# ubc-vision/COTR

Measured on AMD Instinct MI355X. Metric: query-correspondences/sec at 256x512 SBS, 1k queries, higher is better.
Workload: dtype f32

## Files before the change

cotr_amd/_lib.py:

```python
import ctypes
import os

import torch

from .build import LIB, LIB_EXP

c_float_p = ctypes.c_void_p

_PROTOS = {
    'cotr_abi_version': (ctypes.c_int, []),
    'cotr_create': (ctypes.c_int, [ctypes.POINTER(ctypes.c_void_p), ctypes.c_int]),
    'cotr_destroy': (None, [ctypes.c_void_p]),
    'cotr_last_error': (ctypes.c_char_p, [ctypes.c_void_p]),
    'cotr_load_weights': (ctypes.c_int, [ctypes.c_void_p, ctypes.POINTER(ctypes.c_char_p),
                                         ctypes.POINTER(ctypes.c_void_p), ctypes.POINTER(ctypes.c_int64), ctypes.c_int]),
    'cotr_encode': (ctypes.c_int, [ctypes.c_void_p, c_float_p, ctypes.c_int, ctypes.c_void_p]),
    'cotr_backbone': (ctypes.c_int, [ctypes.c_void_p, c_float_p, ctypes.c_int, c_float_p, ctypes.c_void_p]),
    'cotr_backbone_upto': (ctypes.c_int, [ctypes.c_void_p, c_float_p, ctypes.c_int, ctypes.c_int, c_float_p, ctypes.c_void_p]),
    'cotr_decode': (ctypes.c_int, [ctypes.c_void_p, c_float_p, ctypes.c_int, ctypes.c_int, c_float_p, ctypes.c_void_p]),
    'cotr_forward': (ctypes.c_int, [ctypes.c_void_p, c_float_p, c_float_p, ctypes.c_int, ctypes.c_int, c_float_p,
                                    ctypes.c_void_p]),
    'cotr_workspace_bytes': (ctypes.c_int, [ctypes.c_void_p, ctypes.c_int, ctypes.c_int, ctypes.POINTER(ctypes.c_size_t)]),
    'cotr_scratch_bytes': (ctypes.c_int, [ctypes.c_void_p, ctypes.c_int, ctypes.c_int, ctypes.POINTER(ctypes.c_size_t)]),
    'cotr_batch_chunks': (ctypes.c_int, [ctypes.c_void_p, ctypes.c_int, ctypes.c_int, ctypes.c_int, ctypes.POINTER(ctypes.c_int), ctypes.c_int]),
# ... 109 lines not shown
    'cotr_get_knob': (ctypes.c_int, [ctypes.c_void_p, ctypes.c_char_p, ctypes.POINTER(ctypes.c_int), ctypes.POINTER(ctypes.c_int)]),
    'cotr_set_knob': (ctypes.c_int, [ctypes.c_void_p, ctypes.c_char_p, ctypes.c_int]),
    'cotr_check_knob': (ctypes.c_int, [ctypes.c_char_p, ctypes.c_int]),
    'cotr_reset_knobs': (ctypes.c_int, [ctypes.c_void_p]),
    'cotr_is_experimental': (ctypes.c_int, []),
    'cotr_bench_linear': (ctypes.c_int, [c_float_p, c_float_p, c_float_p, c_float_p, ctypes.c_int, ctypes.c_int,
                                         ctypes.c_int, ctypes.c_int, ctypes.c_int, ctypes.POINTER(ctypes.c_float)]),
    'cotr_bench_conv': (ctypes.c_int, [c_float_p, c_float_p, c_float_p, c_float_p, c_float_p] + [ctypes.c_int] * 9 +
                        [ctypes.POINTER(ctypes.c_float)]),
    'cotr_op_linear_cfg': (ctypes.c_int, [c_float_p, c_float_p, c_float_p, c_float_p, ctypes.c_int, c_float_p,
                                          ctypes.c_int, ctypes.c_int, ctypes.c_int, ctypes.c_int, ctypes.c_void_p]),
    'cotr_op_conv_cfg': (ctypes.c_int, [c_float_p, c_float_p, c_float_p, c_float_p, c_float_p, ctypes.c_int, c_float_p] +
                         [ctypes.c_int] * 8 + [ctypes.c_void_p]),
    'cotr_debug_ffn_times': (ctypes.c_int, [ctypes.c_void_p]),
    'cotr_debug_attention_times': (ctypes.c_int, [ctypes.c_void_p]),
    'cotr_gemm_pick_conv': (ctypes.c_int, [ctypes.c_int] * 7),
    'cotr_debug_conv_times': (ctypes.c_int, [c_float_p, c_float_p, c_float_p, c_float_p, c_float_p] + [ctypes.c_int] * 8 +
                              [ctypes.c_void_p, ctypes.c_void_p]),
}

_EXP_PROTOS = {
    'cotr_op_dec_head': (ctypes.c_int, [c_float_p] * 11 + [ctypes.c_int, ctypes.c_int, ctypes.c_int, ctypes.c_void_p]),
    'cotr_op_linear_ln': (ctypes.c_int, [c_float_p] * 7 + [ctypes.c_int, ctypes.c_int, ctypes.c_void_p]),
    'cotr_op_split_h2': (ctypes.c_int, [c_float_p, ctypes.c_void_p, ctypes.c_size_t, ctypes.c_void_p]),
    'cotr_op_unsplit_h2': (ctypes.c_int, [ctypes.c_void_p, c_float_p, ctypes.c_size_t, ctypes.c_void_p]),
    'cotr_op_set_h2_flags': (ctypes.c_int, [ctypes.c_int]),
    'cotr_h2_fallbacks': (ctypes.c_long, []),
    'cotr_op_attention_h2': (ctypes.c_int, [c_float_p, ctypes.c_int, ctypes.c_int, c_float_p, c_float_p, ctypes.c_int, c_float_p, ctypes.c_int,
                                            ctypes.c_int, ctypes.c_int, ctypes.c_int, ctypes.c_void_p]),
}
# ... 88 lines not shown
```

cotr_amd/csrc/api.hip:

```cpp
#include <math.h>
#include <stdio.h>
#include <stdlib.h>
#include <string.h>

#include <algorithm>
#include <map>
#include <string>
#include <vector>

#include <limits.h>

#include "../../include/cotr_hip.h"
#include "common.h"
#include "train.h"

int init_attention_attributes();
void set_ffn_debug_times(unsigned long long* p);
void set_attention_debug_times(unsigned long long* p);

namespace {

constexpr int D = 256, FFN = 1024, TOK = 512, CFEAT = 1024;
constexpr int ENC_CHUNK_MAX = 128;
constexpr int DEC_ROWS = 32768;
constexpr float QSCALE = 0.17677669529663687f;

struct ConvW {
  const float *w, *scale, *bias;
  int cin, cout, k, stride;
};
struct EncW {
  const float *in_w, *in_b, *out_w, *out_b, *l1w, *l1b, *l2w, *l2b, *n1w, *n1b, *n2w, *n2b;
// ... 69 lines not shown
}
KnobSet g_process_knobs = default_knobs();
}
thread_local const KnobSet* cotr_tls_knobs = &g_process_knobs;

struct cotr_ctx {
  int device = 0;
  std::string err;
  KnobSet knobs = default_knobs();
  float* wbuf = nullptr;
  size_t wfloats = 0;
  bool loaded = false;
  std::vector<ConvW> convs;
  struct FusedBlock { const float *w2p = nullptr, *w3p = nullptr, *wdp = nullptr; };
  FusedBlock l1_fused[3];
  const float *ip_w = nullptr, *ip_b = nullptr;
  std::vector<EncW> enc;
  std::vector<DecW> dec;
  const float *kv_w = nullptr, *kv_b = nullptr;
  const float *dn_w = nullptr, *dn_b = nullptr;
  const float* mlp_w[3] = {nullptr, nullptr, nullptr};
  const float* mlp_b[3] = {nullptr, nullptr, nullptr};
  float* pos = nullptr;
  float* tab_qkv = nullptr;
  float* tab_kv = nullptr;
  Arena memkv;
  int enc_B = 0;
  Arena enc_scr, dec_scr;
  std::map<std::string, std::pair<const float*, size_t>> taps;
  bool keep_taps = false;
// ... 414 lines not shown
  h->device = device;
  if (hipMalloc(reinterpret_cast<void**>(&h->pos), (size_t)TOK * D * sizeof(float)) != hipSuccess ||
      launch_pos_table(h->pos, nullptr) != 0 || hipStreamSynchronize(nullptr) != hipSuccess) {
    g_create_error = "building the image position table failed";
    delete h;
    return COTR_ERR_HIP;
  }
  *out = h;
  return COTR_OK;
}

void cotr_destroy(cotr_handle h) {
  if (!h) return;
  DeviceScope scope(h->device);
  (void)hipDeviceSynchronize();
  prof_reset(h);
  if (h->wbuf) (void)hipFree(h->wbuf);
  if (h->pos) (void)hipFree(h->pos);
  for (hipEvent_t ev : {h->ev_fork, h->ev_q, h->ev_mem, h->ev_kv})
    if (ev) (void)hipEventDestroy(ev);
  if (h->side) (void)hipStreamDestroy(h->side);
  for (Arena* a : {&h->memkv, &h->enc_scr, &h->dec_scr})
    if (a->ptr && !a->external) (void)hipFree(a->ptr);
  for (auto& kv : h->tap_store)
    if (kv.second.ptr) (void)hipFree(kv.second.ptr);
  for (auto& st : h->vl_stage) {
    if (st.host) (void)hipHostFree(st.host);
    if (st.ev) (void)hipEventDestroy(st.ev);
  }
  delete h;
// ... 92 lines not shown
      inplanes = planes * 4;
    }
  }
  size_t l1_w2p[3], l1_w3p[3], l1_wdp = 0;
  for (int b = 0; b < 3; ++b) {
    const int c1i = b == 0 ? 1 : 5 + 3 * (b - 1);
    l1_w2p[b] = reserve(36864);
    l1_w3p[b] = reserve(16384);
    bottleneck_pack_w2(&host[convs[c1i + 1].w], &host[l1_w2p[b]]);
    bottleneck_pack_w3(&host[convs[c1i + 2].w], &host[l1_w3p[b]]);
    if (b == 0) {
      l1_wdp = reserve(16384);
      bottleneck_pack_w3(&host[convs[c1i + 3].w], &host[l1_wdp]);
    }
  }
  const size_t ip_w = put("input_proj.weight", (size_t)D * CFEAT), ip_b = put("input_proj.bias", D);

  struct EncOff { size_t v[12]; };
  std::vector<EncOff> enc(n_enc), dec(n_dec);
  for (int i = 0; i < n_enc; ++i) {
    const std::string p = "transformer.encoder.layers." + std::to_string(i) + ".";
    size_t* v = enc[i].v;
    v[0] = put(p + "self_attn.in_proj_weight", (size_t)3 * D * D);
    v[1] = put(p + "self_attn.in_proj_bias", 3 * D);
    v[2] = put(p + "self_attn.out_proj.weight", (size_t)D * D);
    v[3] = put(p + "self_attn.out_proj.bias", D);
    v[4] = put(p + "linear1.weight", (size_t)FFN * D);
    v[5] = put(p + "linear1.bias", FFN);
    v[6] = put(p + "linear2.weight", (size_t)D * FFN);
    v[7] = put(p + "linear2.bias", D);
// ... 46 lines not shown
    h->wbuf = nullptr;
  }
  if (!h->wbuf) {
    HIPCHK(h, hipMalloc(reinterpret_cast<void**>(&h->wbuf), host.size() * sizeof(float)));
    h->wfloats = host.size();
  }
  HIPCHK(h, hipMemcpy(h->wbuf, host.data(), host.size() * sizeof(float), hipMemcpyHostToDevice));
  const float* base = h->wbuf;
  h->convs.clear();
  for (const auto& c : convs) h->convs.push_back({base + c.w, base + c.scale, base + c.bias, c.cin, c.cout, c.k, c.stride});
  for (int b = 0; b < 3; ++b) {
    h->l1_fused[b].w2p = base + l1_w2p[b];
    h->l1_fused[b].w3p = base + l1_w3p[b];
    h->l1_fused[b].wdp = b == 0 ? base + l1_wdp : nullptr;
  }
  h->ip_w = base + ip_w; h->ip_b = base + ip_b;
  h->enc.clear();
  for (const auto& e : enc)
    h->enc.push_back({base + e.v[0], base + e.v[1], base + e.v[2], base + e.v[3], base + e.v[4], base + e.v[5],
                      base + e.v[6], base + e.v[7], base + e.v[8], base + e.v[9], base + e.v[10], base + e.v[11]});
  h->dec.clear();
  for (const auto& e : dec)
    h->dec.push_back({base + e.v[0], base + e.v[1], base + e.v[2], base + e.v[3], base + e.v[4], base + e.v[5],
                      base + e.v[6], base + e.v[7], base + e.v[8], base + e.v[9], base + e.v[10], base + e.v[11]});
  h->kv_w = base + kv_w; h->kv_b = base + kv_b;
  h->dn_w = base + dn_w; h->dn_b = base + dn_b;
  for (int i = 0; i < 3; ++i) { h->mlp_w[i] = base + mw[i]; h->mlp_b[i] = base + mb[i]; }
  h->tab_qkv = h->wbuf + tab_qkv;
  h->tab_kv = h->wbuf + tab_kv;
  for (int l = 0; l < n_enc; ++l)
// ... 1 lines not shown
                       h->tab_qkv + (size_t)l * TOK * 3 * D, TOK, 2 * D, D, nullptr, 3 * D)) return r;
  for (int l = 0; l < n_dec; ++l)
    if (int r = linear(h, h->pos, nullptr, 0, 1, 0, h->kv_w + (size_t)l * 2 * D * D, nullptr, nullptr, 0, 1.f, 0,
                       h->tab_kv + (size_t)l * 2 * D, TOK, D, D, nullptr, n_dec * 2 * D)) return r;
  HIPCHK(h, hipStreamSynchronize(nullptr));
  h->loaded = true;
  h->enc_B = 0;
  return COTR_OK;
}

static int enc_backbone_pass(cotr_ctx* h, const EncBufs& eb, const float* img_c, int Bc, int b0, float* src_out, float* feat_out,
                             int upto, hipStream_t s) {
  int ci = 0;
  if (knob(KN_FUSED_STEM) && !h->keep_taps) {
    const ConvW& c0 = h->convs[ci++];
    KCHK(h, launch_stem_pool(img_c, c0.w, 160, c0.scale, c0.bias, eb.b_pool, Bc, s), "stem_pool");
    prof_mark(h, "stem_pool conv7x7+bn+relu+maxpool", s, 2);
  } else {
    { int r = stem(h, h->convs[ci++], img_c, eb.b_stem, Bc, s); if (r) return r; }
    KCHK(h, launch_maxpool(eb.b_stem, eb.b_pool, Bc, 128, 128, 64, s), "maxpool");
    prof_mark(h, "maxpool", s, 2);
  }
  prof_mark(h, "stem+pool", s);
  if (int r = tap_save(h, "stem", eb.b_stem, ENC_STEM * Bc, s)) return r;
  if (int r = tap_save(h, "pool", eb.b_pool, ENC_POOL * Bc, s)) return r;
  const float* x = eb.b_pool;
  float* outbuf[2] = {eb.b_x, eb.b_y};
  int flip = 0, H = 64, W = 64;
  for (int st = 0; st < 3; ++st) {
    for (int b = 0; b < kStages[st].blocks; ++b) {
      const int stride = (b == 0) ? kStages[st].stride : 1;
// ... 727 lines not shown
  p.A = x; p.lda = Cin; p.W = w; p.C = y; p.ldc = Cout;
  p.scale = scale; p.bias = bias; p.residual = residual; p.ldr = Cout; p.relu = relu;
  return op_ret(launch_gemm(GEMM_CONV, p, static_cast<hipStream_t>(stream)));
}

int cotr_op_stem(const float* img, const float* w, const float* scale, const float* bias, float* y, int B,
                 cotr_stream stream) {
  GemmParams p = base_params();
  p.M = B * 128 * 256; p.N = 64; p.K = 160; p.A = img; p.W = w; p.C = y; p.ldc = 64;
  p.scale = scale; p.bias = bias; p.relu = 1;
  return op_ret(launch_gemm(GEMM_STEM, p, static_cast<hipStream_t>(stream)));
}

int cotr_op_stem_pool(const float* img, const float* w, const float* scale, const float* bias, float* y, int B,
                      cotr_stream stream) {
  return op_ret(launch_stem_pool(img, w, 160, scale, bias, y, B, static_cast<hipStream_t>(stream)));
}

int cotr_op_maxpool(const float* x, float* y, int B, int Hin, int Win, int C, cotr_stream stream) {
  return op_ret(launch_maxpool(x, y, B, Hin, Win, C, static_cast<hipStream_t>(stream)));
}

int cotr_op_attention(const float* q, int ldq, const float* k, const float* v, int ldkv, float* o, int ldo,
                      int nb, int nq, cotr_stream stream) {
  if (init_attention_attributes() != 0) return COTR_ERR_HIP;
  return op_ret(launch_attention(q, ldq, k, v, ldkv, o, ldo, nb, nq, static_cast<hipStream_t>(stream)));
}

int cotr_op_attention_fused(const float* q, int ldq, const float* x, const float* x2, const float* wq, const float* bq,
                            float qscale, const float* k, const float* v, int ldkv, float* o, int ldo, const float* wo,
                            float* part, int nb, int nq, cotr_stream stream) {
// ... 167 lines not shown
  p.A = x; p.lda = Cin; p.W = w; p.C = y; p.ldc = Cout;
  p.scale = scale; p.bias = bias; p.residual = residual; p.ldr = Cout; p.relu = relu;
  return op_ret(launch_gemm_cfg(GEMM_CONV, cfg, p, static_cast<hipStream_t>(stream)));
}

int cotr_debug_ffn_times(unsigned long long* times) {
  set_ffn_debug_times(times);
  return COTR_OK;
}

int cotr_debug_attention_times(unsigned long long* times) {
  set_attention_debug_times(times);
  return COTR_OK;
}

int cotr_gemm_pick_conv(int B, int Hin, int Win, int Cin, int Cout, int ksize, int stride) {
  GemmParams p = base_params();
  const int pad = ksize / 2;
  p.Hin = Hin; p.Win = Win; p.Cin = Cin;
  p.Hout = (Hin + 2 * pad - ksize) / stride + 1;
  p.Wout = (Win + 2 * pad - ksize) / stride + 1;
  p.ksize = ksize; p.stride = stride; p.pad = pad;
  p.M = B * p.Hout * 2 * p.Wout; p.N = Cout; p.K = ksize * ksize * Cin;
  p.lda = Cin; p.ldc = Cout; p.ldr = Cout;
  return gemm_pick_config(GEMM_CONV, p);
}

int cotr_debug_conv_times(const float* x, const float* w, const float* scale, const float* bias, float* y, int B, int Hin, int Win,
                          int Cin, int Cout, int ksize, int stride, int cfg, unsigned long long* times, cotr_stream stream) {
  GemmParams p = base_params();
// ... 192 lines not shown
```

cotr_amd/csrc/bottleneck.hip:

```cpp
#include "common.h"

struct BottleneckParams {
  const float* x;
  float* y;
  const float* w1;
  const float* w2p;
  const float* w3p;
  const float* wdp;
  const float *s1, *b1, *s2, *b2, *s3, *b3, *sd, *bd;
  const float* zeros;
  int B;
};

#define BT_H 64
#define BT_W 64
#define BT_LDT 68

template <int CIN, bool DS>
__global__ __launch_bounds__(512) void bottleneck_kernel(const BottleneckParams p) {
  static_assert(CIN == 64 || CIN == 256, "layer1: 64 (block 0) or 256 input channels");
  static_assert(!DS || CIN == 64, "the downsample branch belongs to block 0");
  constexpr int LDX = CIN + 4;
  constexpr int C4 = CIN / 4;
  constexpr int NX = 64 * C4 / 512;
  extern __shared__ __attribute__((aligned(16))) float smem[];
  float* Xs = smem;
  float* W1s = Xs + 64 * LDX;
  float* T1s = W1s + 64 * LDX;
  float* T2s = T1s + 64 * BT_LDT;
  float* RED = (CIN == 256) ? W1s : T2s + 32 * BT_LDT;

  const int t = threadIdx.x, lane = t & 63;
  const int wave = __builtin_amdgcn_readfirstlane(t >> 6);
  const int l31 = lane & 31, hh = lane >> 5;
  const int bid = blockIdx.x;
  const int tx = bid & 15, ty = (bid >> 4) & 15, b = bid >> 8;
  const int side = tx >> 3, x0 = (tx & 7) * 8, y0 = ty * 4;
  const size_t pair_base = (size_t)b * BT_H * (2 * BT_W);

  f32x4 xr[NX], wr[NX];
#pragma unroll
  for (int i = 0; i < NX; ++i) {
    const int idx = t + 512 * i;
    const int row = idx / C4, c4 = idx % C4;
    const int py = (row * 205) >> 11, px = row - py * 10;
    const int yy = y0 - 1 + py, xx = x0 - 1 + px;
    const bool ok = row < 60 && yy >= 0 && yy < BT_H && xx >= 0 && xx < BT_W;
// ... 12 lines not shown
    for (int j = 0; j < 8; ++j) w3f[j] = w3g[j * 64];
    if constexpr (DS) {
      const f32x4* wdg = reinterpret_cast<const f32x4*>(p.wdp) + (size_t)(wave * 8) * 64 + lane;
#pragma unroll
      for (int j = 0; j < 8; ++j) wdf[j] = wdg[j * 64];
    }
  }
#pragma unroll
  for (int i = 0; i < NX; ++i) {
    const int idx = t + 512 * i;
    const int row = idx / C4, c4 = idx % C4;
    *reinterpret_cast<f32x4*>(&Xs[row * LDX + c4 * 4]) = xr[i];
    *reinterpret_cast<f32x4*>(&W1s[row * LDX + c4 * 4]) = wr[i];
  }
  __syncthreads();

  {
    const int mb = wave & 1, nb = (wave >> 1) & 1, kh = wave >> 2;
    constexpr int NS = CIN / 16;
    f32x16 acc;
#pragma unroll
    for (int r = 0; r < 16; ++r) acc[r] = 0.f;
    const float* ar = &Xs[(32 * mb + l31) * LDX + kh * (CIN / 2) + hh * 4];
    const float* br = &W1s[(32 * nb + l31) * LDX + kh * (CIN / 2) + hh * 4];
#pragma unroll
    for (int j = 0; j < NS; ++j) {
      const f32x4 a = *reinterpret_cast<const f32x4*>(ar + j * 8);
      const f32x4 bb = *reinterpret_cast<const f32x4*>(br + j * 8);
#pragma unroll
      for (int e = 0; e < 4; ++e) acc = __builtin_amdgcn_mfma_f32_32x32x2f32(a[e], bb[e], acc, 0, 0, 0);
// ... 8 lines not shown
      const int ch = 32 * nb + l31;
      const float sc = p.s1[ch], bi = p.b1[ch];
#pragma unroll
      for (int r = 0; r < 16; ++r) {
        const int row = 32 * mb + (r & 3) + 8 * (r >> 2) + 4 * hh;
        const int py = (row * 205) >> 11, px = row - py * 10;
        const int yy = y0 - 1 + py, xx = x0 - 1 + px;
        const bool ok = row < 60 && yy >= 0 && yy < BT_H && xx >= 0 && xx < BT_W;
        float v = acc[r] + RED[((mb * 2 + nb) * 16 + r) * 64 + lane];
        v = fmaf(v, sc, bi);
        v = (v < 0.f) ? 0.f : v;
        T1s[row * BT_LDT + ch] = ok ? v : 0.f;
      }
    }
    __syncthreads();
  }

  {
    f32x16 acc;
#pragma unroll
    for (int r = 0; r < 16; ++r) acc[r] = 0.f;
    const int rowbase = (l31 >> 3) * 10 + (l31 & 7);
#pragma unroll
    for (int i = 0; i < 18; ++i) {
      const int s = 18 * kgB + i;
      const int tap = s >> 3, kc = s & 7;
      const int ky = (tap * 11) >> 5, kx = tap - 3 * ky;
      const f32x4 a = *reinterpret_cast<const f32x4*>(&T1s[(rowbase + ky * 10 + kx) * BT_LDT + kc * 8 + hh * 4]);
#pragma unroll
      for (int e = 0; e < 4; ++e) acc = __builtin_amdgcn_mfma_f32_32x32x2f32(a[e], w2f[i][e], acc, 0, 0, 0);
// ... 3 lines not shown
    __syncthreads();
    const int nb = wave & 1, rg = wave >> 1;
    const int ch = 32 * nb + l31;
    const float sc = p.s2[ch], bi = p.b2[ch];
#pragma unroll
    for (int rr = 0; rr < 4; ++rr) {
      const int r = rg * 4 + rr;
      float v = 0.f;
#pragma unroll
      for (int kg = 0; kg < 4; ++kg) v += RED[((kg * 2 + nb) * 16 + r) * 64 + lane];
      v = fmaf(v, sc, bi);
      v = (v < 0.f) ? 0.f : v;
      T2s[((r & 3) + 8 * (r >> 2) + 4 * hh) * BT_LDT + ch] = v;
    }
    __syncthreads();
  }

  {
    f32x16 acc, accd;
#pragma unroll
    for (int r = 0; r < 16; ++r) acc[r] = accd[r] = 0.f;
#pragma unroll
    for (int j = 0; j < 8; ++j) {
      const f32x4 a = *reinterpret_cast<const f32x4*>(&T2s[l31 * BT_LDT + j * 8 + hh * 4]);
#pragma unroll
      for (int e = 0; e < 4; ++e) acc = __builtin_amdgcn_mfma_f32_32x32x2f32(a[e], w3f[j][e], acc, 0, 0, 0);
    }
    if constexpr (DS) {
      const int crow = ((l31 >> 3) + 1) * 10 + (l31 & 7) + 1;
#pragma unroll
      for (int j = 0; j < 8; ++j) {
        const f32x4 a = *reinterpret_cast<const f32x4*>(&Xs[crow * LDX + j * 8 + hh * 4]);
#pragma unroll
        for (int e = 0; e < 4; ++e) accd = __builtin_amdgcn_mfma_f32_32x32x2f32(a[e], wdf[j][e], accd, 0, 0, 0);
      }
    }
    const int n = 32 * wave + l31;
    const float sc = p.s3[n], bi = p.b3[n];
    float scd = 0.f, bid_ = 0.f;
    if constexpr (DS) { scd = p.sd[n]; bid_ = p.bd[n]; }
#pragma unroll
    for (int r = 0; r < 16; ++r) {
      const int px = (r & 3) + 8 * (r >> 2) + 4 * hh;
      const int oy = px >> 3, ox = px & 7;
      float v = fmaf(acc[r], sc, bi);
      if constexpr (DS) v += fmaf(accd[r], scd, bid_);
      else v += Xs[((oy + 1) * 10 + ox + 1) * LDX + n];
      v = (v < 0.f) ? 0.f : v;
      p.y[(pair_base + (size_t)(y0 + oy) * (2 * BT_W) + side * BT_W + x0 + ox) * 256 + n] = v;
    }
  }
}

template <int CIN>
static constexpr size_t bottleneck_smem() {
  return (size_t)(2 * 64 * (CIN + 4) + 64 * BT_LDT + 32 * BT_LDT + (CIN == 256 ? 0 : 8 * 16 * 64)) * sizeof(float);
}

int launch_bottleneck(const float* x, float* y, int B, int cin, const float* w1, const float* w2p, const float* w3p, const float* wdp,
                      const float* s1, const float* b1, const float* s2, const float* b2, const float* s3, const float* b3,
                      const float* sd, const float* bd, hipStream_t s) {
  if (B <= 0) return 0;
  if (!((cin == 64 && wdp != nullptr) || (cin == 256 && wdp == nullptr))) return -1;
  BottleneckParams p;
  p.x = x; p.y = y; p.w1 = w1; p.w2p = w2p; p.w3p = w3p; p.wdp = wdp;
  p.s1 = s1; p.b1 = b1; p.s2 = s2; p.b2 = b2; p.s3 = s3; p.b3 = b3; p.sd = sd; p.bd = bd;
  p.zeros = gemm_zero_buffer();
  p.B = B;
  if (p.zeros == nullptr) return -2;
  static_assert(bottleneck_smem<256>() <= 163840, "LDS");
  const int grid = B * 256;
  if (cin == 64) {
    static PerDeviceFlag attr_set;
    if (!attr_set.get()) {
      if (hipFuncSetAttribute(reinterpret_cast<const void*>(bottleneck_kernel<64, true>), hipFuncAttributeMaxDynamicSharedMemorySize,
                              (int)bottleneck_smem<64>()) != hipSuccess)
        return -2;
      attr_set.set();
    }
    hipLaunchKernelGGL((bottleneck_kernel<64, true>), dim3(grid), dim3(512), bottleneck_smem<64>(), s, p);
  } else {
    static PerDeviceFlag attr_set;
    if (!attr_set.get()) {
      if (hipFuncSetAttribute(reinterpret_cast<const void*>(bottleneck_kernel<256, false>), hipFuncAttributeMaxDynamicSharedMemorySize,
                              (int)bottleneck_smem<256>()) != hipSuccess)
        return -2;
      attr_set.set();
    }
    hipLaunchKernelGGL((bottleneck_kernel<256, false>), dim3(grid), dim3(512), bottleneck_smem<256>(), s, p);
  }
  return hipGetLastError() == hipSuccess ? 0 : -2;
}

void bottleneck_pack_w2(const float* w2, float* w2p) {
  for (int nb = 0; nb < 2; ++nb)
    for (int kg = 0; kg < 4; ++kg)
      for (int i = 0; i < 18; ++i)
        for (int lane = 0; lane < 64; ++lane)
          for (int e = 0; e < 4; ++e)
            w2p[((((size_t)(nb * 4 + kg) * 18 + i) * 64 + lane) * 4) + e] =
                w2[(size_t)(32 * nb + (lane & 31)) * 576 + (18 * kg + i) * 8 + (lane >> 5) * 4 + e];
}
void bottleneck_pack_w3(const float* w3, float* w3p) {
  for (int w = 0; w < 8; ++w)
    for (int j = 0; j < 8; ++j)
// ... 5 lines not shown
```

cotr_amd/csrc/common.h:

```cpp
#pragma once
#ifdef COTR_EXPERIMENTAL
#include "experimental/gen/common_exp.h"
#else
#include <hip/hip_runtime.h>
#include <stdint.h>

typedef float f32x4 __attribute__((ext_vector_type(4)));
typedef float f32x16 __attribute__((ext_vector_type(16)));

#define LDS_DMA_WAIT_ALL() asm volatile("s_waitcnt vmcnt(0)" ::: "memory")

__device__ __forceinline__ void store_f32x4(float* dst, const f32x4 v, const bool write_through) {
  if (write_through) asm volatile("global_store_dwordx4 %0, %1, off sc1\n\ts_nop 1" ::"v"(dst), "v"(v) : "memory");
  else *reinterpret_cast<f32x4*>(dst) = v;
}

#define COTR_MAX_DEVICES 64
extern thread_local int cotr_tls_device;
static inline int cotr_current_device() {
  if (cotr_tls_device >= 0) return cotr_tls_device;
  int d = 0;
  if (hipGetDevice(&d) != hipSuccess || d < 0 || d >= COTR_MAX_DEVICES) d = 0;
  return d;
}
// ... 184 lines not shown
                           const float* v, int ldkv, const float* wo, const float* bo, const float* residual, const float* ln_w,
                           const float* ln_b, float* Y, const int4* tiles, int ntiles, hipStream_t s);

int launch_layernorm(const float* x, const float* w, const float* b, float* y, int rows, hipStream_t s);
int launch_posenc(const float* pts, float* y, int nb, int nq, int q_total, hipStream_t s);
int launch_pos_table(float* y , hipStream_t s);
int launch_maxpool(const float* x, float* y, int B, int Hin, int Win, int C, hipStream_t s);
int launch_head2(const float* x, const float* w, const float* b, float* y, int nb, int nq, int q_total,
                 hipStream_t s);

constexpr int PAIR_IDX_MAX = 128;
struct PairIdx { int left[PAIR_IDX_MAX], right[PAIR_IDX_MAX]; };
int launch_pack_pairs(const float* images, int M, int m0, int slots, float* out, hipStream_t s);
int launch_gather_pairs(const float* src, const PairIdx& idx, int nb, float* out, hipStream_t s);

int launch_stem_pool(const float* img, const float* w, int wk, const float* scale, const float* bias, float* out, int B,
                     hipStream_t s);

int launch_crop_resize(const uint8_t* img_a, int ha, int wa, const uint8_t* img_b, int hb, int wb,
                       const int32_t* boxes, int n, float* out, int max_size, hipStream_t s);

int launch_dense_cycle(const float* pred, const double* aff, float* maps, int n_pairs, hipStream_t s);
int launch_dense_merge(const float* maps, const int32_t* boxes, int n_pairs, int side, int H, int W, float* flow,
                       float* conf, hipStream_t s);

int launch_resize_f32(const float* src, int Hs, int Ws, int C, float* dst, int Hd, int Wd, hipStream_t s);

int ffn_fused_chunks(int M);
int launch_ffn_fused(const float* X, const float* W1, const float* b1, const float* W2, float* P, int M, int nch, hipStream_t s);
int launch_ln_reduce_post(const float* parts, int np, const float* bias, const float* residual, const float* w, const float* b,
                          const float* post_w, const float* post_b, float* y, int rows, hipStream_t s);
int launch_ln_reduce(const float* parts, int np, const float* bias, const float* residual, const float* w, const float* b,
// ... 19 lines not shown
```

cotr_amd/csrc/stem_pool.hip:

```cpp
#include "common.h"

#define SP_PH 4
#define SP_PW 8
#define SP_CH (2 * SP_PH + 1)
#define SP_CW (2 * SP_PW + 1)
#define SP_NPIX (SP_CH * SP_CW)
#define SP_MB 10
#define SP_IH (2 * SP_CH + 5)
#define SP_IW (2 * SP_CW + 5)
#define SP_KS 37
#define SP_CP 64

typedef float f32x4v __attribute__((ext_vector_type(4)));

__global__ __launch_bounds__(256) void stem_pool_kernel(const float* __restrict__ img, const float* __restrict__ w,
                                                        const float* __restrict__ scale, const float* __restrict__ bias,
                                                        float* __restrict__ out, int wk) {
  __shared__ float patch[3 * SP_IH * SP_IW];
  __shared__ __attribute__((aligned(16))) float ctile[SP_MB * 16 * SP_CP];
  const int t = threadIdx.x, lane = t & 63, wave = t >> 6;
  const int tx = blockIdx.x % (64 / SP_PW), ty = blockIdx.x / (64 / SP_PW);
  const int side = blockIdx.y, b = blockIdx.z;
  const int cy0 = 2 * ty * SP_PH - 1, cx0 = 2 * tx * SP_PW - 1;
  const int iy0 = 2 * cy0 - 3, ix0 = 2 * cx0 - 3;
  const float* src = img + (size_t)b * 3 * 256 * 512 + side * 256;

  constexpr int NLD = (3 * SP_IH * SP_IW + 255) / 256;
  float pv[NLD];
#pragma unroll
  for (int u = 0; u < NLD; ++u) {
    const int i = t + 256 * u;
    const int c = i / (SP_IH * SP_IW), r = i - c * (SP_IH * SP_IW);
    const int py = r / SP_IW, px = r - py * SP_IW;
    const int y = iy0 + py, x = ix0 + px;
    pv[u] = (i < 3 * SP_IH * SP_IW && y >= 0 && y < 256 && x >= 0 && x < 256) ? src[((size_t)c * 256 + y) * 512 + x] : 0.f;
  }
#pragma unroll
  for (int u = 0; u < NLD; ++u)
    if (t + 256 * u < 3 * SP_IH * SP_IW) patch[t + 256 * u] = pv[u];

  const int g = lane >> 4, n = wave * 16 + (lane & 15);
  float wf[SP_KS];
  int koff[SP_KS];
#pragma unroll
  for (int ks = 0; ks < SP_KS; ++ks) {
    const int k = 4 * ks + g;
    wf[ks] = k < 147 ? w[(size_t)n * wk + k] : 0.f;
    const int kk = k < 147 ? k : 0;
    const int c = kk / 49, r = kk - c * 49, ky = r / 7, kx = r - ky * 7;
    koff[ks] = c * (SP_IH * SP_IW) + ky * SP_IW + kx;
  }
  __syncthreads();

  const float sc = scale[n], bi = bias[n];
#pragma unroll 1
  for (int mb = 0; mb < SP_MB; mb += 2) {
    int base[2];
#pragma unroll
    for (int u = 0; u < 2; ++u) {
      int m = (mb + u) * 16 + (lane & 15);
      if (m >= SP_NPIX) m = SP_NPIX - 1;
      const int cy = m / SP_CW, cx = m - cy * SP_CW;
      base[u] = 2 * cy * SP_IW + 2 * cx;
    }
    f32x4v acc0 = {0.f, 0.f, 0.f, 0.f}, acc1 = {0.f, 0.f, 0.f, 0.f};
    float a0[SP_KS], a1[SP_KS];
#pragma unroll
    for (int ks = 0; ks < SP_KS; ++ks) {
      a0[ks] = patch[base[0] + koff[ks]];
      a1[ks] = patch[base[1] + koff[ks]];
    }
#pragma unroll
    for (int ks = 0; ks < SP_KS; ++ks) {
      acc0 = __builtin_amdgcn_mfma_f32_16x16x4f32(a0[ks], wf[ks], acc0, 0, 0, 0);
      acc1 = __builtin_amdgcn_mfma_f32_16x16x4f32(a1[ks], wf[ks], acc1, 0, 0, 0);
    }
#pragma unroll
    for (int r = 0; r < 4; ++r) {
      float v0 = fmaf(acc0[r], sc, bi), v1 = fmaf(acc1[r], sc, bi);
      ctile[(mb * 16 + 4 * g + r) * SP_CP + n] = (v0 < 0.f) ? 0.f : v0;
      ctile[((mb + 1) * 16 + 4 * g + r) * SP_CP + n] = (v1 < 0.f) ? 0.f : v1;
    }
  }
  __syncthreads();

  for (int i = t; i < SP_PH * SP_PW * 16; i += 256) {
    const int c4 = (i & 15) * 4, p = i >> 4;
    const int ly = p / SP_PW, lx = p - ly * SP_PW;
    f32x4v mx = {-INFINITY, -INFINITY, -INFINITY, -INFINITY};
#pragma unroll
    for (int dy = 0; dy < 3; ++dy) {
      const int cyg = cy0 + 2 * ly + dy;
      if (cyg < 0 || cyg >= 128) continue;
#pragma unroll
      for (int dx = 0; dx < 3; ++dx) {
        const int cxg = cx0 + 2 * lx + dx;
        if (cxg < 0 || cxg >= 128) continue;
        const f32x4v v = *reinterpret_cast<const f32x4v*>(&ctile[((2 * ly + dy) * SP_CW + 2 * lx + dx) * SP_CP + c4]);
#pragma unroll
        for (int e = 0; e < 4; ++e) mx[e] = fmaxf(mx[e], v[e]);
      }
    }
    const int oy = ty * SP_PH + ly, ox = side * 64 + tx * SP_PW + lx;
    *reinterpret_cast<f32x4v*>(out + (((size_t)b * 64 + oy) * 128 + ox) * 64 + c4) = mx;
  }
}

int launch_stem_pool(const float* img, const float* w, int wk, const float* scale, const float* bias, float* out, int B,
                     hipStream_t s) {
  if (B <= 0) return 0;
  if (wk < 147) return -1;
  hipLaunchKernelGGL(stem_pool_kernel, dim3((64 / SP_PH) * (64 / SP_PW), 2, B), dim3(256), 0, s, img, w, scale, bias, out, wk);
  return hipGetLastError() == hipSuccess ? 0 : -2;
}
```

include/cotr_hip.h:

```cpp
#ifndef COTR_HIP_H
#define COTR_HIP_H

#include <stddef.h>
#include <stdint.h>

#ifdef __cplusplus
extern "C" {
#endif
#if defined(__GNUC__) || defined(__clang__)
#pragma GCC visibility push(default)
#endif

#define COTR_HIP_ABI_VERSION 2

#define COTR_OK 0
#define COTR_ERR_ARG (-1)
#define COTR_ERR_HIP (-2)
#define COTR_ERR_STATE (-3)
#define COTR_ERR_WEIGHTS (-4)

typedef struct cotr_ctx* cotr_handle;
typedef void* cotr_stream;

int cotr_abi_version(void);
// ... 183 lines not shown
int cotr_op_bottleneck(const float* x, float* y, int B, int cin, const float* w1, const float* w2, const float* w3, const float* wd,
                       const float* s1, const float* b1, const float* s2, const float* b2, const float* s3, const float* b3,
                       const float* sd, const float* bd, cotr_stream stream);
int cotr_bench_linear(const float* x, const float* w, const float* bias, float* y, int M, int N, int K, int cfg,
                      int iters, float* us);
int cotr_bench_conv(const float* x, const float* w, const float* scale, const float* bias, float* y, int B, int Hin,
                    int Win, int Cin, int Cout, int ksize, int stride, int cfg, int iters, float* us);
int cotr_op_linear_cfg(const float* x, const float* w, const float* bias, const float* residual, int relu, float* y,
                       int M, int N, int K, int cfg, cotr_stream stream);
int cotr_op_conv_cfg(const float* x, const float* w, const float* scale, const float* bias, const float* residual,
                     int relu, float* y, int B, int Hin, int Win, int Cin, int Cout, int ksize, int stride, int cfg,
                     cotr_stream stream);

int cotr_debug_ffn_times(unsigned long long* times);
int cotr_debug_attention_times(unsigned long long* times);
int cotr_gemm_pick_conv(int B, int Hin, int Win, int Cin, int Cout, int ksize, int stride);
int cotr_debug_conv_times(const float* x, const float* w, const float* scale, const float* bias, float* y, int B, int Hin, int Win,
                          int Cin, int Cout, int ksize, int stride, int cfg, unsigned long long* times, cotr_stream stream);

int cotr_op_conv_dual_cfg(const float* x, const float* w0, const float* scale0, const float* bias0, int relu0, float* y0, int Cout0,
                          int ksize0, int stride0, const float* w1, const float* scale1, const float* bias1, int relu1, float* y1,
                          int Cout1, int ksize1, int stride1, int B, int Hin, int Win, int Cin, int cfg, cotr_stream stream);

#ifdef COTR_EXPERIMENTAL
int cotr_op_dec_head(const float* x, const float* nw, const float* nb, const float* w0, const float* b0, const float* w1,
                     const float* b1, const float* w2, const float* b2, float* hs, float* out, int nb_pairs, int nq, int q_total,
                     cotr_stream stream);
int cotr_op_linear_ln(const float* x, const float* w, const float* bias, const float* residual, const float* ln_w, const float* ln_b,
                      float* y, int M, int K, cotr_stream stream);
int cotr_op_split_h2(const float* x, void* y, size_t n, cotr_stream stream);
// ... 15 lines not shown
```

Measured before the change: 1.251 million.

## Prepack stem conv weights and software-pipeline LDS patch reads in stem_pool

Stem 7x7 conv weights are prepacked on the host at load time into a per-wave, per-lane layout. Each lane now fetches its weight fragment with one coalesced load, and the per-k offsets become compile-time constants instead of a strided gather with index arithmetic. The weight loads are issued before the patch is written to LDS so they overlap the image load. The MFMA loop is fully unrolled and uses a rotating six-deep register lookahead for patch reads, with schedule barriers, so LDS latency is hidden behind MFMAs at the cost of more registers. Debug timestamp instrumentation is also added to the stem_pool and bottleneck kernels, compiled out by default.

```diff
diff --git a/cotr_amd/_lib.py b/cotr_amd/_lib.py
--- a/cotr_amd/_lib.py
+++ b/cotr_amd/_lib.py
@@ -147,6 +147,9 @@
                          [ctypes.c_int] * 8 + [ctypes.c_void_p]),
     'cotr_debug_ffn_times': (ctypes.c_int, [ctypes.c_void_p]),
     'cotr_debug_attention_times': (ctypes.c_int, [ctypes.c_void_p]),
+    'cotr_debug_stem_pool_times': (ctypes.c_int, [ctypes.c_void_p]),
+    'cotr_debug_bottleneck_times': (ctypes.c_int, [ctypes.c_void_p]),
+    'cotr_op_stem_pack_w': (ctypes.c_int, [ctypes.c_void_p, ctypes.c_int, ctypes.c_void_p]),
     'cotr_gemm_pick_conv': (ctypes.c_int, [ctypes.c_int] * 7),
     'cotr_debug_conv_times': (ctypes.c_int, [c_float_p, c_float_p, c_float_p, c_float_p, c_float_p] + [ctypes.c_int] * 8 +
                               [ctypes.c_void_p, ctypes.c_void_p]),
diff --git a/cotr_amd/csrc/api.hip b/cotr_amd/csrc/api.hip
--- a/cotr_amd/csrc/api.hip
+++ b/cotr_amd/csrc/api.hip
@@ -16,6 +16,8 @@
 
 int init_attention_attributes();
 void set_ffn_debug_times(unsigned long long* p);
+void set_stem_pool_debug_times(unsigned long long* p);
+void set_bottleneck_debug_times(unsigned long long* p);
 void set_attention_debug_times(unsigned long long* p);
 
 namespace {
@@ -115,6 +117,7 @@
   std::vector<ConvW> convs;
   struct FusedBlock { const float *w2p = nullptr, *w3p = nullptr, *wdp = nullptr; };
   FusedBlock l1_fused[3];
+  float* stem_wp = nullptr;
   const float *ip_w = nullptr, *ip_b = nullptr;
   std::vector<EncW> enc;
   std::vector<DecW> dec;
@@ -559,6 +562,7 @@
   if (!h) return;
   DeviceScope scope(h->device);
   (void)hipDeviceSynchronize();
+  if (h->stem_wp) (void)hipFree(h->stem_wp);
   prof_reset(h);
   if (h->wbuf) (void)hipFree(h->wbuf);
   if (h->pos) (void)hipFree(h->pos);
@@ -681,6 +685,8 @@
       bottleneck_pack_w3(&host[convs[c1i + 3].w], &host[l1_wdp]);
     }
   }
+  std::vector<float> stem_wp(STEM_WP_FLOATS);
+  stem_pool_pack_w(&host[convs[0].w], 160, stem_wp.data());
   const size_t ip_w = put("input_proj.weight", (size_t)D * CFEAT), ip_b = put("input_proj.bias", D);
 
   struct EncOff { size_t v[12]; };
@@ -757,6 +763,8 @@
     h->l1_fused[b].w3p = base + l1_w3p[b];
     h->l1_fused[b].wdp = b == 0 ? base + l1_wdp : nullptr;
   }
+  if (!h->stem_wp) HIPCHK(h, hipMalloc(reinterpret_cast<void**>(&h->stem_wp), STEM_WP_FLOATS * sizeof(float)));
+  HIPCHK(h, hipMemcpy(h->stem_wp, stem_wp.data(), STEM_WP_FLOATS * sizeof(float), hipMemcpyHostToDevice));
   h->ip_w = base + ip_w; h->ip_b = base + ip_b;
   h->enc.clear();
   for (const auto& e : enc)
@@ -788,7 +796,7 @@
   int ci = 0;
   if (knob(KN_FUSED_STEM) && !h->keep_taps) {
     const ConvW& c0 = h->convs[ci++];
-    KCHK(h, launch_stem_pool(img_c, c0.w, 160, c0.scale, c0.bias, eb.b_pool, Bc, s), "stem_pool");
+    KCHK(h, launch_stem_pool(img_c, h->stem_wp, c0.scale, c0.bias, eb.b_pool, Bc, s), "stem_pool");
     prof_mark(h, "stem_pool conv7x7+bn+relu+maxpool", s, 2);
   } else {
     { int r = stem(h, h->convs[ci++], img_c, eb.b_stem, Bc, s); if (r) return r; }
@@ -1546,7 +1554,25 @@
 
 int cotr_op_stem_pool(const float* img, const float* w, const float* scale, const float* bias, float* y, int B,
                       cotr_stream stream) {
-  return op_ret(launch_stem_pool(img, w, 160, scale, bias, y, B, static_cast<hipStream_t>(stream)));
+  if (!img || !w || !scale || !bias || !y || B <= 0) return COTR_ERR_ARG;
+  std::vector<float> hw(64 * 160), packed(STEM_WP_FLOATS);
+  if (hipMemcpy(hw.data(), w, hw.size() * 4, hipMemcpyDeviceToHost) != hipSuccess) return COTR_ERR_HIP;
+  stem_pool_pack_w(hw.data(), 160, packed.data());
+  float* dev = nullptr;
+  if (hipMalloc(reinterpret_cast<void**>(&dev), packed.size() * 4) != hipSuccess) return COTR_ERR_HIP;
+  int rc = COTR_ERR_HIP;
+  if (hipMemcpy(dev, packed.data(), packed.size() * 4, hipMemcpyHostToDevice) == hipSuccess) {
+    rc = op_ret(launch_stem_pool(img, dev, scale, bias, y, B, static_cast<hipStream_t>(stream)));
+    if (hipStreamSynchronize(static_cast<hipStream_t>(stream)) != hipSuccess) rc = COTR_ERR_HIP;
+  }
+  (void)hipFree(dev);
+  return rc;
+}
+
+int cotr_op_stem_pack_w(const float* w, int wk, float* wp) {
+  if (!w || !wp || wk < 147) return COTR_ERR_ARG;
+  stem_pool_pack_w(w, wk, wp);
+  return COTR_OK;
 }
 
 int cotr_op_maxpool(const float* x, float* y, int B, int Hin, int Win, int C, cotr_stream stream) {
@@ -1744,6 +1770,15 @@
   return COTR_OK;
 }
 
+int cotr_debug_stem_pool_times(unsigned long long* times) {
+  set_stem_pool_debug_times(times);
+  return COTR_OK;
+}
+int cotr_debug_bottleneck_times(unsigned long long* times) {
+  set_bottleneck_debug_times(times);
+  return COTR_OK;
+}
+
 int cotr_gemm_pick_conv(int B, int Hin, int Win, int Cin, int Cout, int ksize, int stride) {
   GemmParams p = base_params();
   const int pad = ksize / 2;
diff --git a/cotr_amd/csrc/bottleneck.hip b/cotr_amd/csrc/bottleneck.hip
--- a/cotr_amd/csrc/bottleneck.hip
+++ b/cotr_amd/csrc/bottleneck.hip
@@ -10,13 +10,14 @@
   const float *s1, *b1, *s2, *b2, *s3, *b3, *sd, *bd;
   const float* zeros;
   int B;
+  unsigned long long* dbg;
 };
 
 #define BT_H 64
 #define BT_W 64
 #define BT_LDT 68
 
-template <int CIN, bool DS>
+template <int CIN, bool DS, bool DBG = false>
 __global__ __launch_bounds__(512) void bottleneck_kernel(const BottleneckParams p) {
   static_assert(CIN == 64 || CIN == 256, "layer1: 64 (block 0) or 256 input channels");
   static_assert(!DS || CIN == 64, "the downsample branch belongs to block 0");
@@ -31,6 +32,12 @@
   float* RED = (CIN == 256) ? W1s : T2s + 32 * BT_LDT;
 
   const int t = threadIdx.x, lane = t & 63;
+#define BT_STAMP(slot)                                                                 \
+  do {                                                                                 \
+    if constexpr (DBG)                                                                 \
+      if (t == 0) p.dbg[(size_t)blockIdx.x * 8 + (slot)] = wall_clock64();             \
+  } while (0)
+  BT_STAMP(0);
   const int wave = __builtin_amdgcn_readfirstlane(t >> 6);
   const int l31 = lane & 31, hh = lane >> 5;
   const int bid = blockIdx.x;
@@ -73,6 +80,7 @@
     *reinterpret_cast<f32x4*>(&W1s[row * LDX + c4 * 4]) = wr[i];
   }
   __syncthreads();
+  BT_STAMP(1);
 
   {
     const int mb = wave & 1, nb = (wave >> 1) & 1, kh = wave >> 2;
@@ -111,6 +119,7 @@
       }
     }
     __syncthreads();
+    BT_STAMP(2);
   }
 
   {
@@ -144,6 +153,7 @@
       T2s[((r & 3) + 8 * (r >> 2) + 4 * hh) * BT_LDT + ch] = v;
     }
     __syncthreads();
+    BT_STAMP(3);
   }
 
   {
@@ -164,6 +174,10 @@
 #pragma unroll
         for (int e = 0; e < 4; ++e) accd = __builtin_amdgcn_mfma_f32_32x32x2f32(a[e], wdf[j][e], accd, 0, 0, 0);
       }
+    }
+    if constexpr (DBG) {
+      asm volatile("" ::"v"(acc[0]), "v"(accd[0]) : "memory");
+      BT_STAMP(4);
     }
     const int n = 32 * wave + l31;
     const float sc = p.s3[n], bi = p.b3[n];
@@ -179,12 +193,33 @@
       v = (v < 0.f) ? 0.f : v;
       p.y[(pair_base + (size_t)(y0 + oy) * (2 * BT_W) + side * BT_W + x0 + ox) * 256 + n] = v;
     }
-  }
-}
+    if constexpr (DBG) {
+      asm volatile("s_waitcnt vmcnt(0)" ::: "memory");
+      BT_STAMP(5);
+    }
+  }
+#undef BT_STAMP
+}
+
+static thread_local unsigned long long* g_bottleneck_dbg = nullptr;
+void set_bottleneck_debug_times(unsigned long long* p) { g_bottleneck_dbg = p; }
 
 template <int CIN>
 static constexpr size_t bottleneck_smem() {
   return (size_t)(2 * 64 * (CIN + 4) + 64 * BT_LDT + 32 * BT_LDT + (CIN == 256 ? 0 : 8 * 16 * 64)) * sizeof(float);
+}
+
+template <int CIN, bool DS, bool DBG>
+static int launch_bottleneck_as(const BottleneckParams& p, int grid, hipStream_t s) {
+  static PerDeviceFlag attr_set;
+  if (!attr_set.get()) {
+    if (hipFuncSetAttribute(reinterpret_cast<const void*>(bottleneck_kernel<CIN, DS, DBG>), hipFuncAttributeMaxDynamicSharedMemorySize,
+                            (int)bottleneck_smem<CIN>()) != hipSuccess)
+      return -2;
+    attr_set.set();
+  }
+  hipLaunchKernelGGL((bottleneck_kernel<CIN, DS, DBG>), dim3(grid), dim3(512), bottleneck_smem<CIN>(), s, p);
+  return 0;
 }
 
 int launch_bottleneck(const float* x, float* y, int B, int cin, const float* w1, const float* w2p, const float* w3p, const float* wdp,
@@ -197,28 +232,14 @@
   p.s1 = s1; p.b1 = b1; p.s2 = s2; p.b2 = b2; p.s3 = s3; p.b3 = b3; p.sd = sd; p.bd = bd;
   p.zeros = gemm_zero_buffer();
   p.B = B;
+  p.dbg = g_bottleneck_dbg;
   if (p.zeros == nullptr) return -2;
   static_assert(bottleneck_smem<256>() <= 163840, "LDS");
   const int grid = B * 256;
-  if (cin == 64) {
-    static PerDeviceFlag attr_set;
-    if (!attr_set.get()) {
-      if (hipFuncSetAttribute(reinterpret_cast<const void*>(bottleneck_kernel<64, true>), hipFuncAttributeMaxDynamicSharedMemorySize,
-                              (int)bottleneck_smem<64>()) != hipSuccess)
-        return -2;
-      attr_set.set();
-    }
-    hipLaunchKernelGGL((bottleneck_kernel<64, true>), dim3(grid), dim3(512), bottleneck_smem<64>(), s, p);
-  } else {
-    static PerDeviceFlag attr_set;
-    if (!attr_set.get()) {
-      if (hipFuncSetAttribute(reinterpret_cast<const void*>(bottleneck_kernel<256, false>), hipFuncAttributeMaxDynamicSharedMemorySize,
-                              (int)bottleneck_smem<256>()) != hipSuccess)
-        return -2;
-      attr_set.set();
-    }
-    hipLaunchKernelGGL((bottleneck_kernel<256, false>), dim3(grid), dim3(512), bottleneck_smem<256>(), s, p);
-  }
+  int rc;
+  if (cin == 64) rc = p.dbg ? launch_bottleneck_as<64, true, true>(p, grid, s) : launch_bottleneck_as<64, true, false>(p, grid, s);
+  else rc = p.dbg ? launch_bottleneck_as<256, false, true>(p, grid, s) : launch_bottleneck_as<256, false, false>(p, grid, s);
+  if (rc) return rc;
   return hipGetLastError() == hipSuccess ? 0 : -2;
 }
 
diff --git a/cotr_amd/csrc/common.h b/cotr_amd/csrc/common.h
--- a/cotr_amd/csrc/common.h
+++ b/cotr_amd/csrc/common.h
@@ -222,8 +222,9 @@
 int launch_pack_pairs(const float* images, int M, int m0, int slots, float* out, hipStream_t s);
 int launch_gather_pairs(const float* src, const PairIdx& idx, int nb, float* out, hipStream_t s);
 
-int launch_stem_pool(const float* img, const float* w, int wk, const float* scale, const float* bias, float* out, int B,
-                     hipStream_t s);
+int launch_stem_pool(const float* img, const float* wp, const float* scale, const float* bias, float* out, int B, hipStream_t s);
+void stem_pool_pack_w(const float* w , int wk, float* wp );
+constexpr int STEM_WP_FLOATS = 4 * 37 * 64;
 
 int launch_crop_resize(const uint8_t* img_a, int ha, int wa, const uint8_t* img_b, int hb, int wb,
                        const int32_t* boxes, int n, float* out, int max_size, hipStream_t s);
diff --git a/cotr_amd/csrc/stem_pool.hip b/cotr_amd/csrc/stem_pool.hip
--- a/cotr_amd/csrc/stem_pool.hip
+++ b/cotr_amd/csrc/stem_pool.hip
@@ -13,12 +13,28 @@
 
 typedef float f32x4v __attribute__((ext_vector_type(4)));
 
-__global__ __launch_bounds__(256) void stem_pool_kernel(const float* __restrict__ img, const float* __restrict__ w,
+__host__ __device__ constexpr int sp_koff(int k) {
+  return k < 147 ? (k / 49) * (SP_IH * SP_IW) + ((k % 49) / 7) * SP_IW + (k % 7) : 0;
+}
+
+static thread_local unsigned long long* g_stem_dbg = nullptr;
+void set_stem_pool_debug_times(unsigned long long* p) { g_stem_dbg = p; }
+
+template <bool DBG>
+__global__ __launch_bounds__(256) void stem_pool_kernel(const float* __restrict__ img, const float* __restrict__ wp,
                                                         const float* __restrict__ scale, const float* __restrict__ bias,
-                                                        float* __restrict__ out, int wk) {
+                                                        float* __restrict__ out, unsigned long long* __restrict__ dbg) {
   __shared__ float patch[3 * SP_IH * SP_IW];
   __shared__ __attribute__((aligned(16))) float ctile[SP_MB * 16 * SP_CP];
   const int t = threadIdx.x, lane = t & 63, wave = t >> 6;
+#define SP_STAMP(slot)                                                                                                          \
+  do {                                                                                                                          \
+    if constexpr (DBG)                                                                                                          \
+      if (t == 0) dbg[((size_t)(blockIdx.z * 2 + blockIdx.y) * gridDim.x + blockIdx.x) * 16 + (slot)] = wall_clock64();         \
+  } while (0)
+  SP_STAMP(0);
+  if constexpr (DBG)
+    if (t == 0) dbg[((size_t)(blockIdx.z * 2 + blockIdx.y) * gridDim.x + blockIdx.x) * 16 + 12] = clock64();
   const int tx = blockIdx.x % (64 / SP_PW), ty = blockIdx.x / (64 / SP_PW);
   const int side = blockIdx.y, b = blockIdx.z;
   const int cy0 = 2 * ty * SP_PH - 1, cx0 = 2 * tx * SP_PW - 1;
@@ -35,54 +51,76 @@
     const int y = iy0 + py, x = ix0 + px;
     pv[u] = (i < 3 * SP_IH * SP_IW && y >= 0 && y < 256 && x >= 0 && x < 256) ? src[((size_t)c * 256 + y) * 512 + x] : 0.f;
   }
+  const int g = lane >> 4, n = wave * 16 + (lane & 15);
+  float wf[SP_KS];
+#pragma unroll
+  for (int ks = 0; ks < SP_KS; ++ks) wf[ks] = wp[(wave * SP_KS + ks) * 64 + lane];
+  int koff[SP_KS];
+#pragma unroll
+  for (int ks = 0; ks < SP_KS; ++ks)
+    koff[ks] = g == 0 ? sp_koff(4 * ks) : g == 1 ? sp_koff(4 * ks + 1) : g == 2 ? sp_koff(4 * ks + 2) : sp_koff(4 * ks + 3);
+  if constexpr (DBG) {
+    asm volatile("" ::"v"(pv[NLD - 1]) : "memory");
+    SP_STAMP(1);
+    asm volatile("" ::"v"(wf[SP_KS - 1]) : "memory");
+    SP_STAMP(2);
+  }
 #pragma unroll
   for (int u = 0; u < NLD; ++u)
     if (t + 256 * u < 3 * SP_IH * SP_IW) patch[t + 256 * u] = pv[u];
-
-  const int g = lane >> 4, n = wave * 16 + (lane & 15);
-  float wf[SP_KS];
-  int koff[SP_KS];
-#pragma unroll
-  for (int ks = 0; ks < SP_KS; ++ks) {
-    const int k = 4 * ks + g;
-    wf[ks] = k < 147 ? w[(size_t)n * wk + k] : 0.f;
-    const int kk = k < 147 ? k : 0;
-    const int c = kk / 49, r = kk - c * 49, ky = r / 7, kx = r - ky * 7;
-    koff[ks] = c * (SP_IH * SP_IW) + ky * SP_IW + kx;
-  }
   __syncthreads();
+  SP_STAMP(3);
 
   const float sc = scale[n], bi = bias[n];
-#pragma unroll 1
-  for (int mb = 0; mb < SP_MB; mb += 2) {
-    int base[2];
+  int pb[SP_MB];
 #pragma unroll
-    for (int u = 0; u < 2; ++u) {
-      int m = (mb + u) * 16 + (lane & 15);
-      if (m >= SP_NPIX) m = SP_NPIX - 1;
-      const int cy = m / SP_CW, cx = m - cy * SP_CW;
-      base[u] = 2 * cy * SP_IW + 2 * cx;
-    }
-    f32x4v acc0 = {0.f, 0.f, 0.f, 0.f}, acc1 = {0.f, 0.f, 0.f, 0.f};
-    float a0[SP_KS], a1[SP_KS];
+  for (int mb = 0; mb < SP_MB; ++mb) {
+    int m = mb * 16 + (lane & 15);
+    if (m >= SP_NPIX) m = SP_NPIX - 1;
+    const int cy = m / SP_CW, cx = m - cy * SP_CW;
+    pb[mb] = 2 * cy * SP_IW + 2 * cx;
+  }
+  constexpr int SP_LA = 6, SP_STEPS = (SP_MB / 2) * SP_KS;
+  float ra[SP_LA][2];
+#pragma unroll
+  for (int i = 0; i < SP_LA; ++i) {
+    ra[i][0] = patch[pb[0] + koff[i]];
+    ra[i][1] = patch[pb[1] + koff[i]];
+  }
+  f32x4v acc0, acc1;
+#pragma unroll
+  for (int ps = 0; ps < SP_MB / 2; ++ps) {
+    acc0 = f32x4v{0.f, 0.f, 0.f, 0.f};
+    acc1 = f32x4v{0.f, 0.f, 0.f, 0.f};
 #pragma unroll
     for (int ks = 0; ks < SP_KS; ++ks) {
-      a0[ks] = patch[base[0] + koff[ks]];
-      a1[ks] = patch[base[1] + koff[ks]];
+    const int i = ps * SP_KS + ks;
+    acc0 = __builtin_amdgcn_mfma_f32_16x16x4f32(ra[i % SP_LA][0], wf[ks], acc0, 0, 0, 0);
+    acc1 = __builtin_amdgcn_mfma_f32_16x16x4f32(ra[i % SP_LA][1], wf[ks], acc1, 0, 0, 0);
+    if (i + SP_LA < SP_STEPS) {
+      const int pj = (i + SP_LA) / SP_KS, kj = (i + SP_LA) % SP_KS;
+      ra[i % SP_LA][0] = patch[pb[2 * pj] + koff[kj]];
+      ra[i % SP_LA][1] = patch[pb[2 * pj + 1] + koff[kj]];
     }
+    __builtin_amdgcn_sched_barrier(0);
+    if (ks == SP_KS - 1) {
+      const int mb = 2 * ps;
 #pragma unroll
-    for (int ks = 0; ks < SP_KS; ++ks) {
-      acc0 = __builtin_amdgcn_mfma_f32_16x16x4f32(a0[ks], wf[ks], acc0, 0, 0, 0);
-      acc1 = __builtin_amdgcn_mfma_f32_16x16x4f32(a1[ks], wf[ks], acc1, 0, 0, 0);
+      for (int r = 0; r < 4; ++r) {
+        float v0 = fmaf(acc0[r], sc, bi), v1 = fmaf(acc1[r], sc, bi);
+        ctile[(mb * 16 + 4 * g + r) * SP_CP + n] = (v0 < 0.f) ? 0.f : v0;
+        ctile[((mb + 1) * 16 + 4 * g + r) * SP_CP + n] = (v1 < 0.f) ? 0.f : v1;
+      }
+      if constexpr (DBG) {
+        asm volatile("s_waitcnt lgkmcnt(0)" ::: "memory");
+        SP_STAMP(4 + ps);
+      }
+      __builtin_amdgcn_sched_barrier(0);
     }
-#pragma unroll
-    for (int r = 0; r < 4; ++r) {
-      float v0 = fmaf(acc0[r], sc, bi), v1 = fmaf(acc1[r], sc, bi);
-      ctile[(mb * 16 + 4 * g + r) * SP_CP + n] = (v0 < 0.f) ? 0.f : v0;
-      ctile[((mb + 1) * 16 + 4 * g + r) * SP_CP + n] = (v1 < 0.f) ? 0.f : v1;
     }
   }
   __syncthreads();
+  SP_STAMP(9);
 
   for (int i = t; i < SP_PH * SP_PW * 16; i += 256) {
     const int c4 = (i & 15) * 4, p = i >> 4;
@@ -104,12 +142,27 @@
     const int oy = ty * SP_PH + ly, ox = side * 64 + tx * SP_PW + lx;
     *reinterpret_cast<f32x4v*>(out + (((size_t)b * 64 + oy) * 128 + ox) * 64 + c4) = mx;
   }
+  SP_STAMP(10);
+  if constexpr (DBG)
+    if (t == 0) dbg[((size_t)(blockIdx.z * 2 + blockIdx.y) * gridDim.x + blockIdx.x) * 16 + 13] = clock64();
+#undef SP_STAMP
 }
 
-int launch_stem_pool(const float* img, const float* w, int wk, const float* scale, const float* bias, float* out, int B,
-                     hipStream_t s) {
+int launch_stem_pool(const float* img, const float* wp, const float* scale, const float* bias, float* out, int B, hipStream_t s) {
   if (B <= 0) return 0;
-  if (wk < 147) return -1;
-  hipLaunchKernelGGL(stem_pool_kernel, dim3((64 / SP_PH) * (64 / SP_PW), 2, B), dim3(256), 0, s, img, w, scale, bias, out, wk);
+  const dim3 grid((64 / SP_PH) * (64 / SP_PW), 2, B);
+  if (g_stem_dbg != nullptr)
+    hipLaunchKernelGGL(stem_pool_kernel<true>, grid, dim3(256), 0, s, img, wp, scale, bias, out, g_stem_dbg);
+  else
+    hipLaunchKernelGGL(stem_pool_kernel<false>, grid, dim3(256), 0, s, img, wp, scale, bias, out, nullptr);
   return hipGetLastError() == hipSuccess ? 0 : -2;
 }
+
+void stem_pool_pack_w(const float* w, int wk, float* wp) {
+  for (int wave = 0; wave < 4; ++wave)
+    for (int ks = 0; ks < SP_KS; ++ks)
+      for (int lane = 0; lane < 64; ++lane) {
+        const int k = 4 * ks + (lane >> 4);
+        wp[(wave * SP_KS + ks) * 64 + lane] = k < 147 ? w[(size_t)(16 * wave + (lane & 15)) * wk + k] : 0.f;
+      }
+}
diff --git a/include/cotr_hip.h b/include/cotr_hip.h
--- a/include/cotr_hip.h
+++ b/include/cotr_hip.h
@@ -221,6 +221,9 @@
 
 int cotr_debug_ffn_times(unsigned long long* times);
 int cotr_debug_attention_times(unsigned long long* times);
+int cotr_debug_stem_pool_times(unsigned long long* times);
+int cotr_debug_bottleneck_times(unsigned long long* times);
+int cotr_op_stem_pack_w(const float* w, int wk, float* wp);
 int cotr_gemm_pick_conv(int B, int Hin, int Win, int Cin, int Cout, int ksize, int stride);
 int cotr_debug_conv_times(const float* x, const float* w, const float* scale, const float* bias, float* y, int B, int Hin, int Win,
                           int Cin, int Cout, int ksize, int stride, int cfg, unsigned long long* times, cotr_stream stream);
```

Result: no change. 1.250 million (-0.1%).
